# StandeHaas/Hydrodynamic-Limits-of-Active-Particle-Systems-with-Mean-Field-Interactions

Measured on AMD Instinct MI355X. Metric: particle-steps/sec at N=1e5, higher is better.
Workload: dtype f64; 1 GPU; BASELINE config 2: N=100000 particles, L=200000 sites, K=1, reflecting walls, sigma=0.005 (4001-tap table), beta=0.7, dt=0.0125, exclusion on; method=tiles

## Files before the change

hydrodynamic-limits-of-active-particle-systems-with-mean-field-interactions_amd/capi.py:

```python
from __future__ import annotations

import ctypes as C
import importlib.util
import os
import re
import sys

import numpy as np

HERE = os.path.dirname(os.path.abspath(__file__))
LIB_PATH = os.environ.get("APS_LIB") or os.path.join(HERE, "libaps_hip.so")
HEADER_PATH = os.path.join(os.path.dirname(HERE), "include", "aps.h")

APS_OK, APS_ERR_ARG, APS_ERR_HIP, APS_ERR_STATE, APS_ERR_NODEVICE = 0, -1, -2, -3, -4
METHODS = {"auto": 0, "pairs": 1, "lattice": 2, "tiles": 3}
KERNELS = ("pair_accumulate", "propose", "claim", "apply", "plan_tiles", "propose_lattice", "field_update", "tile_step")


class ApsError(RuntimeError):
    def __init__(self, code, text):
        super().__init__(f"libaps_hip error {code}: {text}")
        self.code = code


# ... 74 lines not shown
        "aps_observe_scalars": (C.c_int, [vp, i32, i32, i32, i32, vp, vp]),
        "aps_observe_scalars_all": (C.c_int, [vp, i32, vp, vp, vp]),
        "aps_event_overhead": (C.c_int, [vp, i32, P(dbl)]),
        "aps_observe_structure": (C.c_int, [vp, i32, i32, vp]),
        "aps_observe_bins": (C.c_int, [vp, i32, i32, vp, vp]),
        "aps_rates_from_field": (C.c_int, [vp, i32, vp, vp, vp, i64, vp, vp, vp, vp]),
        "aps_comm_unique_id": (C.c_int, [vp]),
        "aps_comm_init": (C.c_int, [vp, vp]),
        "aps_comm_ranks": (C.c_int, [vp, P(i32)]),
        "aps_owned_sites": (C.c_int, [vp, P(i32), P(i32)]),
        "aps_halo_copy": (C.c_int, [vp, vp]),
        "aps_halo_pack": (C.c_int, [vp, i32, vp, i64, P(i64)]),
        "aps_halo_unpack": (C.c_int, [vp, i32, vp, i64]),
        "aps_halo_info": (C.c_int, [vp, P(i32), P(i32), P(i32)]),
        "aps_comm_selftest": (C.c_int, [vp, i64]),
        "aps_halo_sizes": (C.c_int, [vp, P(i64), P(i64)]),
        "aps_ipc_export": (C.c_int, [vp, vp]),
        "aps_ipc_connect": (C.c_int, [vp, vp, vp]),
        "aps_exchange_kind": (C.c_int, [vp]),
        "aps_set_flip_table": (C.c_int, [vp, vp, i32]),
        "aps_ntt_info": (C.c_int, [vp, P(i32), P(i32), P(dbl), P(i64)]),
        "aps_ntt_launches": (C.c_int, [vp]),
        "aps_ntt_plan": (C.c_int, [i32, i32, i32, i32, P(i32), P(i32), P(i32)]),
        "aps_ntt_blocks": (C.c_int, [vp, P(i32), P(i32)]),
        "aps_tiles_info": (C.c_int, [vp, P(i32), P(i32), P(i32), P(i32)]),
    }
    lenient = os.environ.get("APS_LIB_LENIENT") == "1"
    for name, (res, args) in protos.items():
        if lenient and not hasattr(lib, name):
            continue
        fn = getattr(lib, name)
        fn.restype, fn.argtypes = res, args
    lib._aps_protos = protos
    _lib = lib
    return lib


def _ptr(a):
    return None if a is None else a.ctypes.data_as(C.c_void_p)


class Handle:

    def __init__(self, *, L, K, periodic, sigma_grid, rate_diffusion, rate_active, beta, dt, seed,
                 n_particles, minus_anchor=True, immobilize=True, suppress_flip=True, crowding=False,
                 k_on=0.0, k_off=0.0, k_exit=0.0, anchor_mask=None, device=0, rank=0, world=1,
# ... 274 lines not shown
        tlen, q = C.c_int32(), C.c_int32()
        self._ck(self.lib.aps_get_table(self._h, None, 0, C.byref(tlen), C.byref(q)))
        out = np.zeros(max(tlen.value, 1))
        self._ck(self.lib.aps_get_table(self._h, _ptr(out), len(out), C.byref(tlen), C.byref(q)))
        return out[:tlen.value], q.value

    def resort(self):
        self._ck(self.lib.aps_resort(self._h))


def device_count():
    return load().aps_device_count()


def ntt_plan(L, Rt, primes, max_log2=21):
    lib = load()
    nb, m, bs = C.c_int32(), C.c_int32(), C.c_int32()
    rc = lib.aps_ntt_plan(int(L), int(Rt), int(primes), int(max_log2), C.byref(nb), C.byref(m), C.byref(bs))
    if rc != APS_OK:
        raise ApsError(rc, lib.aps_last_error(None).decode())
    return dict(blocks=nb.value, log2_m=m.value, block_sites=bs.value)


def comm_unique_id() -> bytes:
    lib = load()
    buf = (C.c_uint8 * 128)()
    rc = lib.aps_comm_unique_id(C.cast(buf, C.c_void_p))
    if rc != APS_OK:
        raise ApsError(rc, lib.aps_last_error(None).decode())
    return bytes(buf)
```

hydrodynamic-limits-of-active-particle-systems-with-mean-field-interactions_amd/csrc/aps_common.hpp:

```cpp
#pragma once

#include <hip/hip_runtime.h>
#include <algorithm>
#include <cmath>
#include <cstdint>
#include <vector>

namespace {

__host__ __device__ inline double aps_exp(double x) {
    const double LOG2E = 0x1.71547652b82fep+0, LN2_HI = 0x1.62e42fee00000p-1, LN2_LO = 0x1.a39ef35793c76p-33;
    x = x > 700.0 ? 700.0 : (x < -700.0 ? -700.0 : x);
    const double kf = rint(x * LOG2E);
    double r = fma(-kf, LN2_HI, x);
    r = fma(-kf, LN2_LO, r);
    double p = 0x1.6124613a86d09p-33;
    p = fma(p, r, 0x1.1eed8eff8d898p-29);
    p = fma(p, r, 0x1.ae64567f544e4p-26);
    p = fma(p, r, 0x1.27e4fb7789f5cp-22);
    p = fma(p, r, 0x1.71de3a556c734p-19);
    p = fma(p, r, 0x1.a01a01a01a01ap-16);
    p = fma(p, r, 0x1.a01a01a01a01ap-13);
    p = fma(p, r, 0x1.6c16c16c16c17p-10);
    p = fma(p, r, 0x1.1111111111111p-7);
// ... 58 lines not shown
    const bool held = M.immobilize && !plus && anchored_site && bound;
    if (held) { act = 0.0; hl = 0.0; hr = 0.0; leave = M.k_exit; }
    double diff = hl + hr;
    if (!(plus && open_f)) act = 0.0;
    if (M.crowding) {
        double ff = 1.0 - (double)o_f / (double)K, fl = 1.0 - (double)o_l / (double)K, fr = 1.0 - (double)o_r / (double)K;
        ff = ff < 0.0 ? 0.0 : (ff > 1.0 ? 1.0 : ff);
        fl = fl < 0.0 ? 0.0 : (fl > 1.0 ? 1.0 : fl);
        fr = fr < 0.0 ? 0.0 : (fr > 1.0 ? 1.0 : fr);
        act *= ff;
        hl = M.rate_diffusion * (double)open_l * fl;
        hr = M.rate_diffusion * (double)open_r * fr;
        diff = hl + hr;
    }
    if (held) { diff = 0.0; act = 0.0; }
    Channels c;
    c.bind = (!bound && !plus && anchored_site && occ_self < K) ? M.k_on : 0.0;
    c.unbind = bound ? M.k_off : 0.0;
    c.diff = diff; c.act = act; c.flip = flip; c.leave = leave; c.left = hl; c.right = hr;
    c.total = ((((diff + act) + flip) + c.bind) + c.unbind) + leave;
    return c;
}

inline void weight_table(double sigma_grid, int L_, int K, bool periodic, std::vector<double> &table, int &tlen, int &q_out, int sum_bits = 51) {
    struct { double sigma_grid; int L, K; bool periodic; } p{sigma_grid, L_, K, periodic};
    table.clear();
    q_out = 0;
    if (!(p.sigma_grid > 0.0)) { tlen = 0; table.push_back(0.0); return; }
    const double s2 = p.sigma_grid * p.sigma_grid;
    const int64_t L = p.L;
    const int64_t lw = p.periodic ? L / 2 : (int64_t)(4.0 * p.sigma_grid + 0.5);
    const int64_t tmax = p.periodic ? L / 2 : std::min(lw, L);
    std::vector<double> w((size_t)tmax + 1);
    double wmax = 0.0;
    for (int64_t t = 0; t <= tmax; ++t) {
        double acc = 0.0;
        if (p.periodic) {
            const double a = (double)t;
            acc = aps_exp(-(0.5 * a * a) / s2);
        } else {
            for (int64_t k = 0;; ++k) {
                const int64_t d1 = t + 2 * L * k, d2 = 2 * L * k - t;
                bool any = false;
                if (d1 <= lw) { const double a = (double)d1; acc += aps_exp(-(0.5 * a * a) / s2); any = true; }
                if (k > 0 && d2 <= lw) { const double a = (double)d2; acc += aps_exp(-(0.5 * a * a) / s2); any = true; }
                if (!any) break;
// ... 65 lines not shown
```

hydrodynamic-limits-of-active-particle-systems-with-mean-field-interactions_amd/csrc/aps_hip.hip:

```cpp

#include <hip/hip_runtime.h>
#include <hip/hip_ext.h>
#include <dlfcn.h>
#include <unistd.h>
#include <rccl/rccl.h>
#include <algorithm>
#include <cmath>
#include <cstdint>
#include <cstdio>
#include <cstdlib>
#include <cstring>
#include <numeric>
#include <string>
#include <vector>

#include "aps.h"
#include "aps_common.hpp"
#include "dev_mem.hpp"

namespace {

constexpr uint32_t POS_MASK = 0x07FFFFFFu;
constexpr uint32_t SPIN_BIT = 1u << 27;
constexpr uint32_t BOUND_BIT = 1u << 28;
// ... 2020 lines not shown
template <bool F32>
const void *tl_kernel_f(bool periodic, int RS, bool k1) {
#define TL_PICK(BC, R) (k1 ? (const void *)&tile_loop<BC, R, true, F32> : (const void *)&tile_loop<BC, R, false, F32>)
#define TL_CASE(R) case R: return periodic ? TL_PICK(1, R) : TL_PICK(0, R);
    if (!F32 && (RS == 8 || (RS == 7 && !k1))) return nullptr;
#ifdef APS_DEV_RS
    switch (RS) { TL_CASE(APS_DEV_RS) default: return nullptr; }
#else
    if constexpr (F32) { if (RS == 8) return periodic ? TL_PICK(1, 8) : TL_PICK(0, 8); }
    switch (RS) {
        TL_CASE(1) TL_CASE(2) TL_CASE(3) TL_CASE(4) TL_CASE(5) TL_CASE(6)
        case 7: return k1 ? (periodic ? (const void *)&tile_loop<1, 7, true, F32> : (const void *)&tile_loop<0, 7, true, F32>)
                          : (F32 ? (periodic ? (const void *)&tile_loop<1, 7, false, true> : (const void *)&tile_loop<0, 7, false, true>) : nullptr);
        default: return nullptr;
    }
#endif
#undef TL_CASE
#undef TL_PICK
}
const void *tl_kernel(const aps_handle *h) {
    return h->f32 ? tl_kernel_f<true>(h->p.periodic != 0, h->ts_RS, h->p.K == 1) : tl_kernel_f<false>(h->p.periodic != 0, h->ts_RS, h->p.K == 1);
}

int loop_prepare(aps_handle *h) {
    if (h->loop_state != -2) return APS_OK;
    h->loop_state = 0;
    auto no = [&](const char *why) { h->loop_why = why; return APS_OK; };
    if (!is_tiles(h)) return no("not the tiles formulation");
    if (h->world != 1) return no("sharded handle");
    if (h->ntt_on) return no("field updated by the exact convolution");
    if (!h->ts_table_in_lds) return no("weight table beyond LDS");
    if (!h->model.field_mode) return no("global mean field");
    if (h->p.K == 1 && h->model.immobilize && h->model.k_exit > 0.0) return no("particles can leave the system (one cell per site)");
    if (3 * h->p.K > 32) return no("site capacity above 10");
    if (h->p.L - (int64_t)(h->ts_ntile - 1) * h->ts_own < 3) return no("last tile shorter than three sites");
#ifdef APS_STAMPS
    return no("diagnostic build");
#endif
    const void *fn = tl_kernel(h);
    if (!fn) return no("no kernel for this frame");
    const int64_t need_per_cu = ((int64_t)h->ts_ntile * h->E + h->num_cu - 1) / h->num_cu;
    h->loop_seg = 0;
    size_t lds_total = 0;
    for (int seg : {256, 192, 128, TL_SEG_MIN}) {
        const TlLds lay = tl_lds_layout(h->tlen, h->ts_RS, h->ts_own, h->p.K, ts_wbytes(h), seg);
        if (lay.total > 160 * 1024) continue;
// ... 469 lines not shown
        }
        if ((double)(((int64_t)p->L + 64 * 8 - 1) / (64 * 8)) * h->E > 8.0 * 256.0 && h->tlen <= 4096) h->fu_R = 7;
        if (const char *env = std::getenv("APS_FU_R")) { const int r = std::atoi(env); if (r >= 2 && r <= 8) h->fu_R = r; }
    }
    h->plan_interval = (!p->periodic && !(p->k_exit > 0.0)) ? 8 : 1;
    if (const char *env = std::getenv("APS_PLAN_INTERVAL")) h->plan_interval = std::max(1, std::atoi(env));

    auto die = [&](int code) { g_create_error = h->err; aps_destroy(h); return code; };
    if (hipSetDevice(p->device) != hipSuccess) { h->err = "hipSetDevice failed"; return die(APS_ERR_HIP); }
    if (hipStreamCreateWithFlags(&h->stream, hipStreamNonBlocking) != hipSuccess) { h->err = "hipStreamCreate failed"; return die(APS_ERR_HIP); }
    h->own_stream = true;
    int rc = set_lds_limit(h);
    if (rc) return die(rc);
    const size_t EN = (size_t)h->E * (size_t)h->Npad, EL = (size_t)h->E * (size_t)p->L;
    h->exit_cap = (int)std::max<int64_t>(h->N, 1);
    if ((rc = dev_alloc(h, &h->d_src, EN)) || (rc = dev_alloc(h, &h->d_orig, EN)) || (rc = dev_alloc(h, &h->d_prop_own, EN)) ||
        (rc = dev_alloc(h, &h->d_sp8, EN)) ||
        (rc = dev_alloc(h, &h->d_tinfo, (size_t)h->E * h->ntiles)) ||
        (rc = dev_alloc(h, &h->d_stamps, (size_t)8 * 4096)) ||
        (rc = dev_alloc(h, &h->d_plan, (size_t)h->E * h->ntiles * PLAN_CAP)) || (rc = dev_alloc(h, &h->d_plan_n, (size_t)h->E * h->ntiles)) ||
        (rc = dev_alloc(h, &h->d_accW, EN * MAX_SPLIT)) || (rc = dev_alloc(h, &h->d_accS, EN * MAX_SPLIT)) ||
        (rc = dev_alloc(h, &h->d_occ, EN * MAX_SPLIT)) || (rc = dev_alloc(h, &h->d_pcnt, 2 * EL)) ||
        (rc = dev_alloc(h, &h->d_plist, EL * 2 * p->K)) || (rc = dev_alloc(h, &h->d_table, h->table.size() + ((size_t)1 << h->bshift) + 8192))    ||
        (rc = dev_alloc(h, &h->d_beta, (size_t)h->E)) || (rc = dev_alloc(h, &h->d_gsum, (size_t)4 * h->E)) ||
        (rc = dev_alloc(h, &h->d_exit, (size_t)h->E * h->exit_cap * 3)) || (rc = dev_alloc(h, &h->d_nexit, (size_t)h->E)) ||
        (rc = dev_alloc(h, &h->d_mfield, (size_t)p->L)))
        return die(rc);
    h->d_prop = h->d_prop_own;
    if (h->method == APS_METHOD_LATTICE) {
        if ((rc = dev_alloc(h, &h->d_ws, EL)) || (rc = dev_alloc(h, &h->d_occ_site, EL)) ||
            (rc = dev_alloc(h, &h->d_dcnt, (size_t)h->E * h->nb)) || (rc = dev_alloc(h, &h->d_dep, (size_t)h->E * h->nb * h->dcap)) ||
            (rc = dev_alloc(h, &h->d_stepw, 2)))
            return die(rc);
    }
    if (h->method == APS_METHOD_TILES && h->world > 1 && (h->ts_kx < 1 || h->ts_kx * std::max(h->ts_reach, 1) > h->ts_ntile / h->world ||
                                                         (h->ts_ntile + h->world - 1) / h->world + 2 * (h->ts_kx - 1) * h->ts_reach > h->ts_ntile)) {
        h->err = "tiles, sharded: halo_interval " + std::to_string(h->ts_kx) + " x reach " + std::to_string(h->ts_reach) +
                 " tiles does not fit a rank's tile range (" + std::to_string(h->ts_ntile / h->world) + " tiles)";
        return die(APS_ERR_ARG);
    }
    if (h->method == APS_METHOD_TILES && h->world > 1 && 2 * h->ts_reach + 1 > h->ts_ntile / h->world) {
        h->err = "tiles, sharded: the table's reach (" + std::to_string(h->ts_reach) + " tiles) must stay below half a rank's tile range (" +
                 std::to_string(h->ts_ntile / h->world) + " tiles): fewer ranks or a larger lattice";
        return die(APS_ERR_ARG);
    }
    if (h->method == APS_METHOD_TILES) {
        const size_t ET = (size_t)h->E * h->ts_ntile;
// ... 19 lines not shown
            for (size_t i = 0; i < ti.size(); ++i) ti[i] = (int)std::ldexp(h->table[i], h->q);
            if ((rc = dev_alloc(h, &h->d_table_i, h->table.size() + ((size_t)1 << h->bshift) + 8192)) ||
                (rc = dev_alloc(h, &h->d_wsi[0], EL)) || (rc = dev_alloc(h, &h->d_wsi[1], EL))) return die(rc);
            if (hipMemcpyAsync(h->d_table_i, ti.data(), ti.size() * sizeof(int), hipMemcpyHostToDevice, h->stream) != hipSuccess ||
                hipStreamSynchronize(h->stream) != hipSuccess) { h->err = "integer table upload failed"; return die(APS_ERR_HIP); }
        }
        if ((rc = ntt_setup(h))) return die(rc);
        if (h->world > 1 && (rc = halo_setup(h))) return die(rc);
        const size_t need = ts_lds_layout(h->tlen, h->ts_table_in_lds, h->ts_RS, h->ts_own, p->K, ts_wbytes(h)).total;
        if (need > 160 * 1024) { h->err = "tiles: site capacity too large for the tile kernel's LDS staging"; return die(APS_ERR_ARG); }
        if (need > 48 * 1024 &&
            hipFuncSetAttribute(ts_kernel(p->periodic != 0, h->ts_table_in_lds, h->ts_RS, p->K == 1, h->f32), hipFuncAttributeMaxDynamicSharedMemorySize, (int)need) != hipSuccess) {
            h->err = "hipFuncSetAttribute(tile_step) failed"; return die(APS_ERR_HIP);
        }
    }
    if (p->anchor_mask) {
        if ((rc = dev_alloc(h, &h->d_anchor, (size_t)p->L))) return die(rc);
        if (hipMemcpyAsync(h->d_anchor, p->anchor_mask, (size_t)p->L, hipMemcpyHostToDevice, h->stream) != hipSuccess) { h->err = "anchor upload failed"; return die(APS_ERR_HIP); }
    }
    h->p.anchor_mask = nullptr;
    if (hipMemcpyAsync(h->d_table, h->table.data(), h->table.size() * sizeof(double), hipMemcpyHostToDevice, h->stream) != hipSuccess ||
        hipMemcpyAsync(h->d_beta, h->beta.data(), h->beta.size() * sizeof(double), hipMemcpyHostToDevice, h->stream) != hipSuccess ||
        hipStreamSynchronize(h->stream) != hipSuccess) { h->err = "table upload failed"; return die(APS_ERR_HIP); }
    *out = h;
    return APS_OK;
}

void aps_destroy(aps_handle *h) {
    if (!h) return;
    if (h->stream) (void)hipStreamSynchronize(h->stream);
    if (h->comm && g_rccl.CommDestroy) (void)g_rccl.CommDestroy(h->comm);
    for (hipEvent_t ev : h->events) (void)hipEventDestroy(ev);
    drop_graphs(h);
    if (h->cap_stream) (void)hipStreamDestroy(h->cap_stream);
    for (void *q : h->ipc_opened) if (q) (void)hipIpcCloseMemHandle(q);
    for (hipEvent_t ev : h->loop_ev) if (ev) (void)hipEventDestroy(ev);
    h->mem.free_all();
    if (h->own_stream && h->stream) (void)hipStreamDestroy(h->stream);
    delete h;
}

int aps_set_stream(aps_handle *h, void *hip_stream) {
    if (!h) return APS_ERR_ARG;
    HIP_TRY(h, hipStreamSynchronize(h->stream));
    if (h->own_stream && h->stream) { HIP_TRY(h, hipStreamDestroy(h->stream)); h->own_stream = false; }
    h->stream = reinterpret_cast<hipStream_t>(hip_stream);
// ... 385 lines not shown
    return APS_OK;
}

int aps_ntt_info(aps_handle *h, int32_t *on, int32_t *log2_m, double *prof_ms, int64_t *prof_launches) {
    if (!h) return APS_ERR_ARG;
    if (on) *on = h->ntt_on ? 1 : 0;
    if (log2_m) *log2_m = h->ntt_on ? h->ntt.m : 0;
    if (prof_ms) *prof_ms = h->prof_ntt_ms;
    if (prof_launches) *prof_launches = h->prof_ntt_n;
    return APS_OK;
}
int aps_ntt_plan(int32_t L, int32_t Rt, int32_t primes, int32_t max_log2, int32_t *blocks, int32_t *log2_m, int32_t *block_sites) {
    if (L < 2 || L > (1 << 25) || Rt < 0 || (primes != 1 && primes != 2)) {
        g_create_error = "aps_ntt_plan: 2 <= L <= 2^25, Rt >= 0, primes 1 or 2";
        return APS_ERR_ARG;
    }
    int nb, m, bs;
    ntt_plan_blocks(L, Rt, primes, max_log2, nb, m, bs);
    if (blocks) *blocks = nb;
    if (log2_m) *log2_m = m;
    if (block_sites) *block_sites = bs;
    return APS_OK;
}
int aps_ntt_blocks(aps_handle *h, int32_t *blocks, int32_t *block_sites) {
    if (!h) return APS_ERR_ARG;
    if (blocks) *blocks = h->ntt_on ? h->ntt.nb : 0;
    if (block_sites) *block_sites = h->ntt_on ? h->ntt.bs : 0;
    return APS_OK;
}
int aps_ntt_launches(aps_handle *h) {
    if (!h || !h->ntt_on) return 0;
    return h->ntt_fused ? 3 : h->ntt.a2 > 0 ? 5 : 3;
}

int aps_mark_reference(aps_handle *h, int32_t e) {
    if (!h) return APS_ERR_ARG;
    if (e < 0 || e >= h->E) return fail(h, APS_ERR_ARG, "aps_mark_reference: bad ensemble");
    if (h->n_set[(size_t)e] < 0) return fail(h, APS_ERR_STATE, "aps_mark_reference: no state uploaded for this ensemble");
    { int rc_ = sync_slots(h); if (rc_) return rc_; }
    int rc;
    if (!h->d_ref && (rc = dev_alloc(h, &h->d_ref, (size_t)h->E * h->Npad))) return rc;
    if (h->ref_set.empty()) h->ref_set.assign((size_t)h->E, 0);
    HIP_TRY(h, hipMemcpyAsync(h->d_ref + (size_t)e * h->Npad, h->d_src + (size_t)e * h->Npad, (size_t)h->Npad * 4, hipMemcpyDeviceToDevice, h->stream));
    HIP_TRY(h, hipStreamSynchronize(h->stream));
    h->ref_set[(size_t)e] = 1;
    return APS_OK;
// ... 311 lines not shown
            h->ipc_peer[side] = static_cast<char *>(ptr);
        }
        for (int par = 0; par < 2; ++par) h->ipc_peer_off[side][par] = (size_t)b[side].land_off[par][side];
    }
    h->ipc_on = true;
    return APS_OK;
}

int aps_set_flip_table(aps_handle *h, const double *table, int32_t n) {
    if (!h) return APS_ERR_ARG;
    HIP_TRY(h, hipStreamSynchronize(h->stream));
    if (h->graphs_built_f[0] || h->graphs_built_f[1]) drop_graphs(h);
    h->mem.release(h->d_flip_tab);
    h->d_flip_tab = nullptr;
    h->model.flip_tab = nullptr; h->model.flip_n = 0;
    if (table) {
        if (n < 1 || n > (1 << 24)) return fail(h, APS_ERR_ARG, "aps_set_flip_table: n must be in [1, 2^24]");
        for (int64_t i = 0; i < 2 * ((int64_t)n + 1); ++i)
            if (!(table[i] >= 0.0) || !std::isfinite(table[i])) return fail(h, APS_ERR_ARG, "aps_set_flip_table: rates must be finite and >= 0");
        HIP_TRY(h, h->mem.alloc(&h->d_flip_tab, (size_t)2 * ((size_t)n + 1)));
        HIP_TRY(h, hipMemcpy(h->d_flip_tab, table, (size_t)2 * ((size_t)n + 1) * sizeof(double), hipMemcpyHostToDevice));
        h->model.flip_tab = h->d_flip_tab; h->model.flip_n = n;
    }
    if (h->d_model) HIP_TRY(h, hipMemcpy(h->d_model, &h->model, sizeof(Model), hipMemcpyHostToDevice));
    return APS_OK;
}

int aps_tiles_info(aps_handle *h, int32_t *frame_sites, int32_t *owned_sites, int32_t *n_tiles, int32_t *table_in_lds) {
    if (!h) return APS_ERR_ARG;
    if (!is_tiles(h)) return fail(h, APS_ERR_STATE, "aps_tiles_info: not a tiles handle");
    if (frame_sites) *frame_sites = 64 * h->ts_RS;
    if (owned_sites) *owned_sites = h->ts_own;
    if (n_tiles) *n_tiles = h->ts_ntile;
    if (table_in_lds) *table_in_lds = h->ts_table_in_lds ? 1 : 0;
    return APS_OK;
}

int aps_exchange_kind(aps_handle *h) { return !h ? APS_ERR_ARG : (h->ipc_on ? 2 : (h->comm ? 1 : 0)); }

int aps_owned_sites(aps_handle *h, int32_t *lo, int32_t *hi) {
    if (!h) return APS_ERR_ARG;
    const bool sharded_sites = is_tiles(h) && h->world > 1;
    if (lo) *lo = sharded_sites ? h->own_lo : 0;
    if (hi) *hi = sharded_sites ? h->own_hi : h->p.L;
    return APS_OK;
}
// ... 250 lines not shown
```

hydrodynamic-limits-of-active-particle-systems-with-mean-field-interactions_amd/csrc/tile_loop.hpp:

```cpp
#pragma once

constexpr int TL_SEG_MIN = 88;
constexpr int TL_NG = 2;
#ifndef TL_MIN_WAVES
#define TL_MIN_WAVES 2
#endif
constexpr int TL_ABORT = 31;

struct LoopArgs {
    TileArgs a;
    unsigned long long step0;
    int nsteps;
    uint32_t tag0;
    int rec, drec;
    int seg;
    unsigned long long *xrec;
    unsigned *abort_dev, *abort_host;
    unsigned long long timeout_ticks;
#ifdef APS_LOOP_DEBUG
    uint32_t *dbg;
#endif
};

struct TlLds { size_t seg, cells, cells2, props, occ, misc, plist, fw, fs, tab, total; };
__host__ __device__ inline TlLds tl_lds_layout(int tlen, int RS, int own, int K, int wbytes, int seg) {
    TlLds l;
    const size_t TS = 64 * (size_t)RS, ncell = (TS + 2) * K;
    auto up = [](size_t v, size_t a) { return (v + a - 1) / a * a; };
    l.seg = 0;
    l.cells = l.seg + (size_t)FU_WAVES * 4 * (seg + 4) * sizeof(uint32_t);
    l.cells2 = up(l.cells + ncell * 4, 8);
    l.props = up(l.cells2 + (K == 1 ? 0 : ncell * 4), 8);
    l.occ = up(l.props + TS * K, 8);
    l.misc = up(l.occ + TS + 2, 8);
    l.plist = l.misc + 128;
    l.fw = up(l.plist + TS * (size_t)K * 8, 16);
    l.fs = l.fw + TS * wbytes;
    l.tab = up(l.fs + TS * wbytes, 16);
    l.total = l.tab + (size_t)ts_table_chunks(tlen, RS, own, wbytes) * 1024;
    return l;
}

typedef __attribute__((address_space(1))) unsigned long long tl_gu64;
typedef __attribute__((address_space(1))) unsigned tl_gu32;

__device__ __forceinline__ void tl_store_granule(unsigned long long *p, uint32_t tag, uint32_t word) {
    __hip_atomic_store((tl_gu64 *)p, ((unsigned long long)tag << 32) | word, __ATOMIC_RELAXED, __HIP_MEMORY_SCOPE_AGENT);
}
__device__ __forceinline__ unsigned long long tl_load_granule(const unsigned long long *p) {
    return __hip_atomic_load((tl_gu64 *)p, __ATOMIC_RELAXED, __HIP_MEMORY_SCOPE_AGENT);
}

__device__ __forceinline__ void tl_lds_add(double *p, double v) { unsafeAtomicAdd(p, v); }
__device__ __forceinline__ void tl_lds_add(int *p, int v) { atomicAdd(p, v); }

template <int BC, int RS, bool K1, bool F32>
__global__ __launch_bounds__(FU_THREADS, TL_MIN_WAVES) void tile_loop(const LoopArgs la, const void *__restrict__ table_v) {
    using W = typename TsField<F32>::w_t;
    using WS = typename TsField<F32>::ws_t;
    constexpr int SH = TsField<F32>::SH, WB = (int)sizeof(W);
    constexpr bool TAB_LDS = true;
    const TileArgs &a = la.a;
    const W *__restrict__ table_g = reinterpret_cast<const W *>(table_v);
    constexpr int TS = 64 * RS, NOLD = (TS + FU_THREADS - 1) / FU_THREADS;
    constexpr int NSLOT = 16, GB = FU_WAVES * 4;
    const int SEG = la.seg;
    extern __shared__ double lds[];
    const int L = a.L, K = K1 ? 1 : a.K, OWN = a.own;
    const TlLds lay = tl_lds_layout(a.tlen, RS, OWN, K, WB, la.seg);
    char *lds_c = reinterpret_cast<char *>(lds);
    uint32_t *seg_all = reinterpret_cast<uint32_t *>(lds_c + lay.seg);
    uint32_t *cellL = reinterpret_cast<uint32_t *>(lds_c + lay.cells);
    uint32_t *cellN = reinterpret_cast<uint32_t *>(lds_c + lay.cells2);
    uint8_t *propL = reinterpret_cast<uint8_t *>(lds_c + lay.props);
    uint8_t *occL = reinterpret_cast<uint8_t *>(lds_c + lay.occ);
    int *misc = reinterpret_cast<int *>(lds_c + lay.misc);
    uint2 *plist = reinterpret_cast<uint2 *>(lds_c + lay.plist);
    W *fieldW = reinterpret_cast<W *>(lds_c + lay.fw), *fieldS = reinterpret_cast<W *>(lds_c + lay.fs);
    W *tab = reinterpret_cast<W *>(lds_c + lay.tab);
    const int t = threadIdx.x, lane = t & 63, wave = __builtin_amdgcn_readfirstlane(t >> 6), e = blockIdx.y;
    const int tile = (int)blockIdx.x;
    const int own0 = tile * OWN, own_n = min(OWN, L - own0), nfr = own_n + 4;
    const int x0 = own0 - 2;
    const int x0c = max(x0, 0), x1c = min(x0 + nfr - 1, L - 1);
    const int Rt = a.tlen - 1;
    if (__hip_atomic_load((tl_gu32 *)la.abort_dev, __ATOMIC_RELAXED, __HIP_MEMORY_SCOPE_AGENT)) {
        if (t == 0) __hip_atomic_store(la.abort_host, 1u, __ATOMIC_RELAXED, __HIP_MEMORY_SCOPE_SYSTEM);
        return;
    }
    int n_iter = la.nsteps;
    {
        const unsigned stall = la.abort_dev[1];
        if (stall && (int)(stall >> 16) - 1 == tile && e == 0) n_iter = min(n_iter, (int)(stall & 0xFFFFu));
    }
    const uint32_t *__restrict__ cell_e = a.cell_in + (size_t)e * L * K;
    const WS *__restrict__ ws_e = reinterpret_cast<const WS *>(a.ws_in) + (size_t)e * L;
    const uint32_t *__restrict__ dcnt_e = a.dcnt_in + (size_t)e * a.ntile;
    const uint32_t *__restrict__ dep_e = a.dep_in + (size_t)e * a.ntile * a.dcap;
    uint32_t tbase = 0;
    {
        typedef __attribute__((address_space(3))) W lds_w;
        tbase = (uint32_t)(size_t)(lds_w *)tab;
    }
    if (t < 32) misc[t] = 0;
    {
        const int nchunk = ts_table_chunks(a.tlen, RS, OWN, WB);
        const char *srct = reinterpret_cast<const char *>(table_g) + lane * 16;
        for (int c = wave; c < nchunk; c += FU_WAVES) {
            const uint32_t m0v = (uint32_t)__builtin_amdgcn_readfirstlane((int)(tbase + (uint32_t)c * 1024u));
            asm volatile("s_mov_b32 m0, %0\n\tglobal_load_lds_dwordx4 %1, off" :: "s"(m0v), "v"(srct + c * 1024) : "memory");
        }
    }
    const double beta = a.beta[e];
    auto frame_site = [&](int i) -> int {
        if (i < -1 || i > nfr) return -1;
        int s = x0 + i;
        if (BC == 1) { s %= L; if (s < 0) s += L; return s; }
        return (s < 0 || s >= L) ? -1 : s;
    };
    const int ncell = (TS + 2) * K;
    for (int c = t; c < ncell; c += FU_THREADS) {
        const int s = frame_site(c / K - 1);
        const uint32_t v = cell_e[(unsigned)max(s, 0) * (unsigned)K + (unsigned)(c % K)];
        cellL[c] = s >= 0 ? v : CELL_EMPTY;
        if (!K1) cellN[c] = CELL_EMPTY;
    }
#pragma unroll
    for (int r = 0; r < NOLD; ++r) {
        const int xi = r * FU_THREADS + t;
        if (xi < TS) {
            const int s = xi < nfr ? frame_site(xi) : -1;
            WS o = ws_e[(unsigned)max(s, 0)];
            if (s < 0) { o.x = 0; o.y = 0; }
            fieldW[xi] = o.x; fieldS[xi] = o.y;
        }
    }
// ... 63 lines not shown
#define TLSTAMP(k)
#endif
    unsigned long long xg[TL_NG], xh = 0;
#pragma unroll
    for (int g = 0; g < TL_NG; ++g) xg[g] = 0;
    const int h_side = lane >> 5, h_i = lane & 31;
    const int h_nb = h_side ? nb_r : nb_l;
    const bool h_act = wave == FU_WAVES - 1 && h_i < 3 * K && h_nb >= 0;
    auto bucket_of = [&](int j, bool &ok) -> int {
        const int bi = j * GB + sub * FU_WAVES + wave;
        ok = j < ngroups && bi < nbk;
        int b = b0 + (ok ? bi : 0);
        if (b >= a.ntile) b -= a.ntile;
        return b;
    };
    for (int it = 0; it < n_iter; ++it) {
        const unsigned long long step = la.step0 + (unsigned long long)it;
        const uint32_t tag_in = la.tag0 + (uint32_t)it, tag_out = tag_in + 1u;
        const bool first = it == 0, last = it + 1 == la.nsteps;
        const unsigned long long *rec_in = la.xrec + ((size_t)((it + 1) & 1) * a.E * a.ntile + rec_e) * la.rec;
        unsigned long long *rec_out = la.xrec + ((size_t)(it & 1) * a.E * a.ntile + rec_e + tile) * la.rec;
        int *dcount = misc + (it & 1), *pcount = misc + 2 + (it & 1);
        bool gave_up = false;
        const int n0 = *pcount;
        uint2 mine = make_uint2(0u, CELL_EMPTY);
        uint32_t rx[4] = {0u, 0u, 0u, 0u};
        if (t < n0) {
            mine = plist[t];
            philox4x32_10((uint32_t)step, (uint32_t)(step >> 32), mine.y & CELL_ID, (uint32_t)(a.ens_base + e), a.seed_lo, a.seed_hi, rx);
        }
        TLSTAMP(2)
        auto spin_check = [&](unsigned &spins, unsigned long long &t_w) -> bool {
            __builtin_amdgcn_s_sleep(1);
            if ((++spins & 63u) != 0u) return false;
            const bool other = __hip_atomic_load((tl_gu32 *)la.abort_dev, __ATOMIC_RELAXED, __HIP_MEMORY_SCOPE_AGENT) != 0;
            const unsigned long long now = __builtin_amdgcn_s_memrealtime();
            if (!t_w) t_w = now;
            if (!other && now - t_w <= la.timeout_ticks) return false;
            if (!other && lane == 0) {
                __hip_atomic_store((tl_gu32 *)la.abort_dev, 1u, __ATOMIC_RELAXED, __HIP_MEMORY_SCOPE_AGENT);
                __hip_atomic_store(la.abort_host, 1u, __ATOMIC_RELAXED, __HIP_MEMORY_SCOPE_SYSTEM);
            }
            gave_up = true;
            return true;
        };
        auto wait_granule = [&](const unsigned long long *p, bool active) -> uint32_t {
            unsigned long long x = 0, t_w = 0;
            for (unsigned spins = 0;;) {
                if (active) x = tl_load_granule(p);
                if (!__ballot(active && (uint32_t)(x >> 32) != tag_in)) break;
                if (spin_check(spins, t_w)) break;
            }
// ... 6 lines not shown
#pragma unroll
                for (int g = 0; g < TL_NG; ++g) {
                    bool ok;
                    const int b = bucket_of(g, ok);
                    if (ok && (uint32_t)(xg[g] >> 32) != tag_in) {
                        xg[g] = tl_load_granule(rec_in + (size_t)b * la.rec + slot);
                        bad |= (uint32_t)(xg[g] >> 32) != tag_in;
                    }
                }
                if (h_act && (uint32_t)(xh >> 32) != tag_in) {
                    xh = tl_load_granule(rec_in + (size_t)h_nb * la.rec + la.drec + (h_side ? 0 : 3 * K) + h_i);
                    bad |= (uint32_t)(xh >> 32) != tag_in;
                }
                if (!__ballot(bad)) break;
                if (spin_check(spins, t_w)) break;
            }
            if (wave == FU_WAVES - 1 && !gave_up) {
                const uint32_t v = h_act ? (uint32_t)xh : CELL_EMPTY;
                const int hs = h_i / K, hk = h_i - hs * K, pos = (h_side ? own_n + 2 : -1) + hs;
                if (h_act) cellL[(h_side ? (own_n + 3) * K : 0) + h_i] = v;
                const unsigned long long mo = __ballot(h_act && v != CELL_EMPTY);
                if (h_i < 3 * K && hk == 0 && h_nb >= 0) occL[pos + 1] = (uint8_t)__popcll((mo >> (h_side * 32 + hs * K)) & ((1ull << K) - 1ull));
                const bool hp = h_act && v != CELL_EMPTY && pos >= 0 && pos < nfr;
                const unsigned long long mh = __ballot(hp);
                if (hp) plist[n0 + __builtin_amdgcn_mbcnt_hi((uint32_t)(mh >> 32), __builtin_amdgcn_mbcnt_lo((uint32_t)mh, 0u))] = make_uint2((uint32_t)pos | ((uint32_t)hk << 16), v);
                if (lane == 0) misc[4 + (it & 1)] = __popcll(mh);
            }
        }
        TLSTAMP(0)
        W accP[RS], accM[RS], accF[RS], accWi[RS], accSi[RS];
#pragma unroll
        for (int r = 0; r < RS; ++r) accP[r] = accM[r] = accF[r] = accWi[r] = accSi[r] = 0;
        uint32_t *shl = seg_all;
        const int CAP = (FU_WAVES * 4 * (SEG + 4) / 4) & ~3;
        unsigned long long *shcnt = reinterpret_cast<unsigned long long *>(misc + 8 + 2 * (it & 1));
        auto sweep_now = [&](unsigned long long m, const uint32_t word, const int cls) {
            while (m) {
                const int src_lane = __builtin_ctzll(m);
                m &= m - 1;
                const uint32_t e1 = (uint32_t)__builtin_amdgcn_readlane((int)word, src_lane);
                if (BC == 0) {
                    if (cls == 0) ts_one_abs<RS, 0, F32>(e1, x8, tb, accP);
                    else if (cls == 1) ts_one_abs<RS, 0, F32>(e1, x8, tb, accM);
                    else if (cls == 2) ts_one_abs<RS, 1, F32>(e1, x8, tb, accF);
                    else ts_image_group<TAB_LDS, RS, F32>(make_uint4(e1, DEP_NULL | ((uint32_t)x0c + TS_BIAS), DEP_NULL | ((uint32_t)x0c + TS_BIAS), DEP_NULL | ((uint32_t)x0c + TS_BIAS)),
                                                          x8, tb, table_g, tlen8, L8, accWi, accSi);
                } else {
                    const uint4 q = make_uint4(e1, DEP_NULL | ((uint32_t)null_site + TS_BIAS), DEP_NULL | ((uint32_t)null_site + TS_BIAS), DEP_NULL | ((uint32_t)null_site + TS_BIAS));
                    if (cls == 0) ts_group<1, TAB_LDS, RS, 0, F32>(q, x8, tb, table_g, tlen8, L8, accP);
// ... 121 lines not shown
            if (nI) {
                const uint32_t nulli = DEP_NULL | ((uint32_t)x0c + TS_BIAS);
                const uint4 *l4 = reinterpret_cast<const uint4 *>(shl + 3 * CAP);
#pragma unroll 1
                for (int g = rot & 3; g < (nI + 3) >> 2; g += FU_WAVES) {
                    uint4 q = l4[g];
                    if (4 * g + 1 >= nI) q.y = nulli;
                    if (4 * g + 2 >= nI) q.z = nulli;
                    if (4 * g + 3 >= nI) q.w = nulli;
                    ts_image_group<TAB_LDS, RS, F32>(q, x8, tb, table_g, tlen8, L8, accWi, accSi);
                }
            }
        }
        TLSTAMP(10)
#pragma unroll
        for (int r = 0; r < RS; ++r) {
            const W dw = (accP[r] + accM[r]) + accWi[r], ds = ((accP[r] - accM[r]) + accF[r]) + accSi[r];
            if (dw != 0) tl_lds_add(&fieldW[r * 64 + lane], dw);
            if (ds != 0) tl_lds_add(&fieldS[r * 64 + lane], ds);
        }
        TLSTAMP(11)
        __syncthreads();
        TLSTAMP(7)
        {
            const Model M = *a.model;
            const int n_part = n0 + misc[4 + (it & 1)];
            auto propose_one = [&](const uint2 pc, const uint32_t (&x)[4]) {
                const int pos = (int)(pc.x & 0xFFFFu), k = (int)(pc.x >> 16);
                const int s = frame_site(pos);
                const bool anch = a.anchor ? a.anchor[s] != 0 : false;
                propL[pos * K + k] = decide_proposal(M, anch, s, (pc.y & CELL_PLUS) ? 1 : -1, (pc.y & CELL_BOUND) != 0,
                                                     clip_field((double)fieldS[pos], (double)fieldW[pos]), beta, occL[pos + 1], occL[pos], occL[pos + 2], x);
            };
            if (t < n_part) {
                if (t >= n0) {
                    mine = plist[t];
                    philox4x32_10((uint32_t)step, (uint32_t)(step >> 32), mine.y & CELL_ID, (uint32_t)(a.ens_base + e), a.seed_lo, a.seed_hi, rx);
                }
                propose_one(mine, rx);
            }
            for (int j = FU_THREADS + t; j < n_part; j += FU_THREADS) {
                const uint2 pc = plist[j];
                uint32_t x[4];
                philox4x32_10((uint32_t)step, (uint32_t)(step >> 32), pc.y & CELL_ID, (uint32_t)(a.ens_base + e), a.seed_lo, a.seed_hi, x);
                propose_one(pc, x);
            }
        }
        __syncthreads();
        TLSTAMP(3)
        auto rank_at = [&](int j, uint32_t id) -> int {
            int n = 0;
            for (int k = 0; k < K; ++k) {
                const uint32_t cl_ = cellL[j * K + k], cr_ = cellL[(j + 2) * K + k];
                const int el = propL[(j - 1) * K + k] & 7, er = propL[(j + 1) * K + k] & 7;
                n += (cl_ != CELL_EMPTY && (el == EV_RIGHT || el == EV_FWD) && (cl_ & CELL_ID) < id);
                n += (cr_ != CELL_EMPTY && er == EV_LEFT && (cr_ & CELL_ID) < id);
            }
            return n;
        };
        auto cap_at = [&](int j) -> int { const int c = K - (int)occL[j + 1]; return c < 1 ? 1 : (c > 32 ? 32 : c); };
        auto put_deposit = [&](int kd, uint32_t d) { if (last) dep_o[kd] = d; else tl_store_granule(rec_out + kd, tag_out, d); };
        auto log_exit = [&](const uint32_t c, const int s) {
            const TileRare R = *a.rare;
            const unsigned kx = atomicAdd(&R.n_exit[e], 1u);
            if ((int)kx < R.exit_cap) {
                double *row = R.exit_log + ((size_t)e * R.exit_cap + kx) * 3;
                row[0] = (double)step; row[1] = (double)s; row[2] = (double)(c & CELL_ID);
            }
// ... 95 lines not shown
                    if (last) cell_o[(unsigned)frame_site(xi) * (unsigned)K + (unsigned)k] = c;
                    else {
                        if (io < 3) tl_store_granule(rec_out + la.drec + io * K + k, tag_out, c);
                        if (io >= own_n - 3) tl_store_granule(rec_out + la.drec + 3 * K + (io - (own_n - 3)) * K + k, tag_out, c);
                    }
                }
                if (!last) append(mine_site && c != CELL_EMPTY, xi, k, c, pnext);
            }
            if (mine_site) {
                occL[xi + 1] = (uint8_t)newn[r];
                if (last) {
                    WS f; f.x = fieldW[xi]; f.y = fieldS[xi];
                    reinterpret_cast<WS *>(a.ws_out)[(size_t)e * L + (unsigned)frame_site(xi)] = f;
                }
            }
        }
        if (!last && t < NSLOT) {
            const int idx = count + t;
            if (idx < (count / NSLOT + 1) * NSLOT && idx < la.drec) tl_store_granule(rec_out + idx, tag_out, DEP_NULL);
        }
        for (int i = t; i < (TS * K + 3) / 4; i += FU_THREADS) reinterpret_cast<uint32_t *>(propL)[i] = 0u;
        if (t == 0) {
            misc[(it + 1) & 1] = 0;
            misc[2 + (it & 1)] = 0; misc[4 + (it & 1)] = 0;
            misc[8 + 2 * (it & 1)] = 0; misc[9 + 2 * (it & 1)] = 0;
            if (last) {
                a.dcnt_out[(size_t)e * a.ntile + tile] = (uint32_t)count;
                if (tile == 0 && e == 0) a.stepw[(a.par + la.nsteps) & 1] = la.step0 + (unsigned long long)la.nsteps;
            }
        }
        if (!last) {
            const unsigned long long *rn = la.xrec + ((size_t)(it & 1) * a.E * a.ntile + rec_e) * la.rec;
#pragma unroll
            for (int g = 0; g < TL_NG; ++g) {
                bool ok;
                const int b = bucket_of(g, ok);
                xg[g] = ok ? tl_load_granule(rn + (size_t)b * la.rec + slot) : 0ull;
            }
            xh = h_act ? tl_load_granule(rn + (size_t)h_nb * la.rec + la.drec + (h_side ? 0 : 3 * K) + h_i) : 0ull;
        }
        TLSTAMP(5)
        __syncthreads();
    }
#ifdef APS_LOOP_STAMPS
    if (lane == 0 && tile < 512 && e == 0) {
        unsigned long long *o = a.rare->stamps + ((size_t)tile * FU_WAVES + wave) * 16;
        for (int k = 0; k < 12; ++k) o[k] = st_acc[k];
        o[6] = __builtin_amdgcn_s_memtime() - st_begin;
        o[1] = st_acc[8] + st_acc[9] + st_acc[10] + st_acc[11];
    }
#endif
}
```

include/aps.h:

```cpp
#ifndef APS_H
#define APS_H

#include <stdint.h>

#ifdef __cplusplus
extern "C" {
#endif

#define APS_OK 0
#define APS_ERR_ARG (-1)
#define APS_ERR_HIP (-2)
#define APS_ERR_STATE (-3)
#define APS_ERR_NODEVICE (-4)

typedef struct aps_handle aps_handle;

typedef struct aps_params {
    int32_t L;
    int32_t K;
    int32_t periodic;
    int32_t minus_anchor;
    int32_t immobilize;
    int32_t suppress_flip;
    int32_t crowding;
// ... 92 lines not shown

int aps_get_exits(aps_handle *h, int32_t ensemble, double *rows3, int64_t cap_rows, int64_t *n_rows);

int aps_get_table(aps_handle *h, double *out, int32_t cap, int32_t *tlen, int32_t *q);

int aps_resort(aps_handle *h);

int aps_step_timed(aps_handle *h, int64_t nsteps, double *kernel_ms, int64_t *launches, double *work);

int aps_step_info(aps_handle *h, int64_t *graph_steps, int64_t *single_steps);

int aps_set_flip_table(aps_handle *h, const double *table, int32_t n);

int aps_ntt_info(aps_handle *h, int32_t *on, int32_t *log2_m, double *prof_ms, int64_t *prof_launches);
int aps_ntt_plan(int32_t L, int32_t Rt, int32_t primes, int32_t max_log2, int32_t *blocks, int32_t *log2_m, int32_t *block_sites);
int aps_ntt_blocks(aps_handle *h, int32_t *blocks, int32_t *block_sites);
int aps_ntt_launches(aps_handle *h);

int aps_tiles_info(aps_handle *h, int32_t *frame_sites, int32_t *owned_sites, int32_t *n_tiles, int32_t *table_in_lds);

int aps_set_resident_loop(aps_handle *h, int32_t on);
int aps_loop_info(aps_handle *h, int64_t *loop_steps, int32_t *state, char *why, int32_t why_len);
int aps_step_loop_timed(aps_handle *h, int64_t nsteps, double *kernel_ms, int64_t *loop_steps);

int aps_copy_bandwidth(aps_handle *h, int64_t nbytes, int32_t reps, double *gbytes_per_s);

int aps_event_overhead(aps_handle *h, int32_t reps, double *ms_per_pair);

int aps_step_profile(aps_handle *h, int64_t nsteps, double *ms8, int64_t *launches8);

#ifdef __cplusplus
}
#endif
#endif
```

Before: 8.252 billion particle-steps/s.

## Prefilter particles by an upper-bound fire probability before proposing moves

```diff
diff --git a/hydrodynamic-limits-of-active-particle-systems-with-mean-field-interactions_amd/capi.py b/hydrodynamic-limits-of-active-particle-systems-with-mean-field-interactions_amd/capi.py
--- a/hydrodynamic-limits-of-active-particle-systems-with-mean-field-interactions_amd/capi.py
+++ b/hydrodynamic-limits-of-active-particle-systems-with-mean-field-interactions_amd/capi.py
@@ -120,6 +120,7 @@
         "aps_ntt_info": (C.c_int, [vp, P(i32), P(i32), P(dbl), P(i64)]),
         "aps_ntt_launches": (C.c_int, [vp]),
         "aps_ntt_plan": (C.c_int, [i32, i32, i32, i32, P(i32), P(i32), P(i32)]),
+        "aps_p_fire_bound": (C.c_int, [C.c_double] * 7 + [vp, i32, P(C.c_double)]),
         "aps_ntt_blocks": (C.c_int, [vp, P(i32), P(i32)]),
         "aps_tiles_info": (C.c_int, [vp, P(i32), P(i32), P(i32), P(i32)]),
     }
@@ -440,6 +441,17 @@
     return dict(blocks=nb.value, log2_m=m.value, block_sites=bs.value)
 
 
+def p_fire_bound(rate_diffusion, rate_active, k_on, k_off, k_exit, dt, beta, flip_table=None):
+    lib = load()
+    tab = None if flip_table is None else np.ascontiguousarray(flip_table, dtype=np.float64)
+    out = C.c_double()
+    rc = lib.aps_p_fire_bound(float(rate_diffusion), float(rate_active), float(k_on), float(k_off), float(k_exit), float(dt), float(beta),
+                              None if tab is None else _ptr(tab), 0 if tab is None else tab.shape[1] - 1, C.byref(out))
+    if rc != APS_OK:
+        raise ApsError(rc, lib.aps_last_error(None).decode())
+    return out.value
+
+
 def comm_unique_id() -> bytes:
     lib = load()
     buf = (C.c_uint8 * 128)()
diff --git a/hydrodynamic-limits-of-active-particle-systems-with-mean-field-interactions_amd/csrc/aps_common.hpp b/hydrodynamic-limits-of-active-particle-systems-with-mean-field-interactions_amd/csrc/aps_common.hpp
--- a/hydrodynamic-limits-of-active-particle-systems-with-mean-field-interactions_amd/csrc/aps_common.hpp
+++ b/hydrodynamic-limits-of-active-particle-systems-with-mean-field-interactions_amd/csrc/aps_common.hpp
@@ -104,6 +104,19 @@
     return c;
 }
 
+inline double p_fire_bound(const Model &M, double beta, const double *flip_host) {
+    auto pos = [](double v) { return v < 0.0 ? 0.0 : v; };
+    double f_max = std::exp(std::fabs(beta));
+    if (M.flip_n > 0 && flip_host) {
+        f_max = 0.0;
+        for (int64_t i = 0; i < 2 * ((int64_t)M.flip_n + 1); ++i) f_max = std::max(f_max, flip_host[i]);
+    }
+    const double t_max = 2.0 * pos(M.rate_diffusion) + pos(M.rate_active) + f_max + pos(M.k_on) + pos(M.k_off) + pos(M.k_exit);
+    const double margin = 1.0 + 0x1.0p-40;
+    const double p_hi = (1.0 - std::exp(-(t_max * pos(M.dt) * margin))) * margin + 0x1.0p-50;
+    return p_hi < 1.0 ? p_hi : 2.0;
+}
+
 inline void weight_table(double sigma_grid, int L_, int K, bool periodic, std::vector<double> &table, int &tlen, int &q_out, int sum_bits = 51) {
     struct { double sigma_grid; int L, K; bool periodic; } p{sigma_grid, L_, K, periodic};
     table.clear();
diff --git a/hydrodynamic-limits-of-active-particle-systems-with-mean-field-interactions_amd/csrc/aps_hip.hip b/hydrodynamic-limits-of-active-particle-systems-with-mean-field-interactions_amd/csrc/aps_hip.hip
--- a/hydrodynamic-limits-of-active-particle-systems-with-mean-field-interactions_amd/csrc/aps_hip.hip
+++ b/hydrodynamic-limits-of-active-particle-systems-with-mean-field-interactions_amd/csrc/aps_hip.hip
@@ -2066,6 +2066,13 @@
     return h->f32 ? tl_kernel_f<true>(h->p.periodic != 0, h->ts_RS, h->p.K == 1) : tl_kernel_f<false>(h->p.periodic != 0, h->ts_RS, h->p.K == 1);
 }
 
+int upload_p_hi(aps_handle *h, const double *flip_host) {
+    std::vector<double> p_hi((size_t)h->E);
+    for (int e = 0; e < h->E; ++e) p_hi[(size_t)e] = p_fire_bound(h->model, h->beta[(size_t)e], flip_host);
+    HIP_TRY(h, hipMemcpy(h->d_beta + h->E, p_hi.data(), p_hi.size() * sizeof(double), hipMemcpyHostToDevice));
+    return APS_OK;
+}
+
 int loop_prepare(aps_handle *h) {
     if (h->loop_state != -2) return APS_OK;
     h->loop_state = 0;
@@ -2581,7 +2588,7 @@
         (rc = dev_alloc(h, &h->d_accW, EN * MAX_SPLIT)) || (rc = dev_alloc(h, &h->d_accS, EN * MAX_SPLIT)) ||
         (rc = dev_alloc(h, &h->d_occ, EN * MAX_SPLIT)) || (rc = dev_alloc(h, &h->d_pcnt, 2 * EL)) ||
         (rc = dev_alloc(h, &h->d_plist, EL * 2 * p->K)) || (rc = dev_alloc(h, &h->d_table, h->table.size() + ((size_t)1 << h->bshift) + 8192))    ||
-        (rc = dev_alloc(h, &h->d_beta, (size_t)h->E)) || (rc = dev_alloc(h, &h->d_gsum, (size_t)4 * h->E)) ||
+        (rc = dev_alloc(h, &h->d_beta, (size_t)2 * h->E))    || (rc = dev_alloc(h, &h->d_gsum, (size_t)4 * h->E)) ||
         (rc = dev_alloc(h, &h->d_exit, (size_t)h->E * h->exit_cap * 3)) || (rc = dev_alloc(h, &h->d_nexit, (size_t)h->E)) ||
         (rc = dev_alloc(h, &h->d_mfield, (size_t)p->L)))
         return die(rc);
@@ -2647,6 +2654,7 @@
     if (hipMemcpyAsync(h->d_table, h->table.data(), h->table.size() * sizeof(double), hipMemcpyHostToDevice, h->stream) != hipSuccess ||
         hipMemcpyAsync(h->d_beta, h->beta.data(), h->beta.size() * sizeof(double), hipMemcpyHostToDevice, h->stream) != hipSuccess ||
         hipStreamSynchronize(h->stream) != hipSuccess) { h->err = "table upload failed"; return die(APS_ERR_HIP); }
+    if ((rc = upload_p_hi(h, nullptr))) return die(rc);
     *out = h;
     return APS_OK;
 }
@@ -3078,6 +3086,15 @@
     if (block_sites) *block_sites = bs;
     return APS_OK;
 }
+int aps_p_fire_bound(double rate_diffusion, double rate_active, double k_on, double k_off, double k_exit, double dt, double beta,
+                     const double *flip_table, int32_t flip_n, double *p_hi) {
+    if (!p_hi || flip_n < 0 || (flip_n > 0 && !flip_table)) { g_create_error = "aps_p_fire_bound: null argument"; return APS_ERR_ARG; }
+    Model M{};
+    M.rate_diffusion = rate_diffusion; M.rate_active = rate_active; M.k_on = k_on; M.k_off = k_off; M.k_exit = k_exit; M.dt = dt;
+    M.flip_n = flip_n;
+    *p_hi = p_fire_bound(M, beta, flip_table);
+    return APS_OK;
+}
 int aps_ntt_blocks(aps_handle *h, int32_t *blocks, int32_t *block_sites) {
     if (!h) return APS_ERR_ARG;
     if (blocks) *blocks = h->ntt_on ? h->ntt.nb : 0;
@@ -3435,6 +3452,7 @@
         HIP_TRY(h, hipMemcpy(h->d_flip_tab, table, (size_t)2 * ((size_t)n + 1) * sizeof(double), hipMemcpyHostToDevice));
         h->model.flip_tab = h->d_flip_tab; h->model.flip_n = n;
     }
+    if (int rc = upload_p_hi(h, table)) return rc;
     if (h->d_model) HIP_TRY(h, hipMemcpy(h->d_model, &h->model, sizeof(Model), hipMemcpyHostToDevice));
     return APS_OK;
 }
diff --git a/hydrodynamic-limits-of-active-particle-systems-with-mean-field-interactions_amd/csrc/tile_loop.hpp b/hydrodynamic-limits-of-active-particle-systems-with-mean-field-interactions_amd/csrc/tile_loop.hpp
--- a/hydrodynamic-limits-of-active-particle-systems-with-mean-field-interactions_amd/csrc/tile_loop.hpp
+++ b/hydrodynamic-limits-of-active-particle-systems-with-mean-field-interactions_amd/csrc/tile_loop.hpp
@@ -4,6 +4,9 @@
 constexpr int TL_NG = 2;
 #ifndef TL_MIN_WAVES
 #define TL_MIN_WAVES 2
+#endif
+#ifndef TL_ROT_SHIFT
+#define TL_ROT_SHIFT 8
 #endif
 constexpr int TL_ABORT = 31;
 
@@ -22,7 +25,7 @@
 #endif
 };
 
-struct TlLds { size_t seg, cells, cells2, props, occ, misc, plist, fw, fs, tab, total; };
+struct TlLds { size_t seg, cells, cells2, props, occ, misc, plist, sv_x, sv_pc, fw, fs, tab, total; };
 __host__ __device__ inline TlLds tl_lds_layout(int tlen, int RS, int own, int K, int wbytes, int seg) {
     TlLds l;
     const size_t TS = 64 * (size_t)RS, ncell = (TS + 2) * K;
@@ -34,7 +37,9 @@
     l.occ = up(l.props + TS * K, 8);
     l.misc = up(l.occ + TS + 2, 8);
     l.plist = l.misc + 128;
-    l.fw = up(l.plist + TS * (size_t)K * 8, 16);
+    l.sv_x = up(l.plist + TS * (size_t)K * 8, 16);
+    l.sv_pc = l.sv_x + TS * (size_t)K * 16;
+    l.fw = up(l.sv_pc + TS * (size_t)K * 8, 16);
     l.fs = l.fw + TS * wbytes;
     l.tab = up(l.fs + TS * wbytes, 16);
     l.total = l.tab + (size_t)ts_table_chunks(tlen, RS, own, wbytes) * 1024;
@@ -76,6 +81,8 @@
     uint8_t *occL = reinterpret_cast<uint8_t *>(lds_c + lay.occ);
     int *misc = reinterpret_cast<int *>(lds_c + lay.misc);
     uint2 *plist = reinterpret_cast<uint2 *>(lds_c + lay.plist);
+    uint4 *sv_x = reinterpret_cast<uint4 *>(lds_c + lay.sv_x);
+    uint2 *sv_pc = reinterpret_cast<uint2 *>(lds_c + lay.sv_pc);
     W *fieldW = reinterpret_cast<W *>(lds_c + lay.fw), *fieldS = reinterpret_cast<W *>(lds_c + lay.fs);
     W *tab = reinterpret_cast<W *>(lds_c + lay.tab);
     const int t = threadIdx.x, lane = t & 63, wave = __builtin_amdgcn_readfirstlane(t >> 6), e = blockIdx.y;
@@ -112,6 +119,8 @@
         }
     }
     const double beta = a.beta[e];
+    const double p_hi = a.beta[a.E + e];
+    const int prop_wave = (tile + (tile >> TL_ROT_SHIFT)) & (FU_WAVES - 1);
     auto frame_site = [&](int i) -> int {
         if (i < -1 || i > nfr) return -1;
         int s = x0 + i;
@@ -221,12 +230,30 @@
         unsigned long long *rec_out = la.xrec + ((size_t)(it & 1) * a.E * a.ntile + rec_e + tile) * la.rec;
         int *dcount = misc + (it & 1), *pcount = misc + 2 + (it & 1);
         bool gave_up = false;
-        const int n0 = *pcount;
-        uint2 mine = make_uint2(0u, CELL_EMPTY);
-        uint32_t rx[4] = {0u, 0u, 0u, 0u};
-        if (t < n0) {
-            mine = plist[t];
-            philox4x32_10((uint32_t)step, (uint32_t)(step >> 32), mine.y & CELL_ID, (uint32_t)(a.ens_base + e), a.seed_lo, a.seed_hi, rx);
+        const int n0 = __builtin_amdgcn_readfirstlane(*pcount);
+        auto draw = [&](const uint2 pc, uint32_t (&x)[4]) -> bool {
+            philox4x32_10((uint32_t)step, (uint32_t)(step >> 32), pc.y & CELL_ID, (uint32_t)(a.ens_base + e), a.seed_lo, a.seed_hi, x);
+            const double u0 = ((double)(x[0] >> 5) * 67108864.0 + (double)(x[1] >> 6)) * 0x1.0p-53;
+            return u0 < p_hi;
+        };
+        auto survive = [&](bool sv, const uint2 pc, const uint32_t (&x)[4]) {
+            const unsigned long long mm = __ballot(sv);
+            const int cnt_u = __popcll(mm);
+            int base = 0;
+            if (lane == 0 && cnt_u) base = atomicAdd(misc + 6, cnt_u);
+            base = __builtin_amdgcn_readfirstlane(base);
+            if (sv) {
+                const int i = base + (int)__builtin_amdgcn_mbcnt_hi((uint32_t)(mm >> 32), __builtin_amdgcn_mbcnt_lo((uint32_t)mm, 0u));
+                sv_pc[i] = pc; sv_x[i] = make_uint4(x[0], x[1], x[2], x[3]);
+            }
+        };
+        for (int j0 = wave * 64; j0 < n0; j0 += FU_THREADS) {
+            const int j = j0 + lane;
+            uint2 pc = make_uint2(0u, CELL_EMPTY);
+            uint32_t x[4] = {0u, 0u, 0u, 0u};
+            bool sv = false;
+            if (j < n0) { pc = plist[j]; sv = draw(pc, x); }
+            survive(sv, pc, x);
         }
         TLSTAMP(2)
         auto spin_check = [&](unsigned &spins, unsigned long long &t_w) -> bool {
@@ -279,9 +306,11 @@
                 const unsigned long long mo = __ballot(h_act && v != CELL_EMPTY);
                 if (h_i < 3 * K && hk == 0 && h_nb >= 0) occL[pos + 1] = (uint8_t)__popcll((mo >> (h_side * 32 + hs * K)) & ((1ull << K) - 1ull));
                 const bool hp = h_act && v != CELL_EMPTY && pos >= 0 && pos < nfr;
-                const unsigned long long mh = __ballot(hp);
-                if (hp) plist[n0 + __builtin_amdgcn_mbcnt_hi((uint32_t)(mh >> 32), __builtin_amdgcn_mbcnt_lo((uint32_t)mh, 0u))] = make_uint2((uint32_t)pos | ((uint32_t)hk << 16), v);
-                if (lane == 0) misc[4 + (it & 1)] = __popcll(mh);
+                const uint2 hpc = make_uint2((uint32_t)pos | ((uint32_t)hk << 16), v);
+                uint32_t hx[4] = {0u, 0u, 0u, 0u};
+                bool hsv = false;
+                if (hp) hsv = draw(hpc, hx);
+                survive(hsv, hpc, hx);
             }
         }
         TLSTAMP(0)
@@ -449,9 +478,10 @@
         TLSTAMP(11)
         __syncthreads();
         TLSTAMP(7)
-        {
+        const int nsv = __builtin_amdgcn_readfirstlane(misc[6]);
+        const int sv0 = ((wave - prop_wave) & (FU_WAVES - 1)) * 64;
+        if (sv0 < nsv) {
             const Model M = *a.model;
-            const int n_part = n0 + misc[4 + (it & 1)];
             auto propose_one = [&](const uint2 pc, const uint32_t (&x)[4]) {
                 const int pos = (int)(pc.x & 0xFFFFu), k = (int)(pc.x >> 16);
                 const int s = frame_site(pos);
@@ -459,18 +489,10 @@
                 propL[pos * K + k] = decide_proposal(M, anch, s, (pc.y & CELL_PLUS) ? 1 : -1, (pc.y & CELL_BOUND) != 0,
                                                      clip_field((double)fieldS[pos], (double)fieldW[pos]), beta, occL[pos + 1], occL[pos], occL[pos + 2], x);
             };
-            if (t < n_part) {
-                if (t >= n0) {
-                    mine = plist[t];
-                    philox4x32_10((uint32_t)step, (uint32_t)(step >> 32), mine.y & CELL_ID, (uint32_t)(a.ens_base + e), a.seed_lo, a.seed_hi, rx);
-                }
-                propose_one(mine, rx);
-            }
-            for (int j = FU_THREADS + t; j < n_part; j += FU_THREADS) {
-                const uint2 pc = plist[j];
-                uint32_t x[4];
-                philox4x32_10((uint32_t)step, (uint32_t)(step >> 32), pc.y & CELL_ID, (uint32_t)(a.ens_base + e), a.seed_lo, a.seed_hi, x);
-                propose_one(pc, x);
+            for (int j = sv0 + lane; j < nsv; j += FU_THREADS) {
+                const uint4 x4 = sv_x[j];
+                const uint32_t x[4] = {x4.x, x4.y, x4.z, x4.w};
+                propose_one(sv_pc[j], x);
             }
         }
         __syncthreads();
@@ -612,7 +634,7 @@
         for (int i = t; i < (TS * K + 3) / 4; i += FU_THREADS) reinterpret_cast<uint32_t *>(propL)[i] = 0u;
         if (t == 0) {
             misc[(it + 1) & 1] = 0;
-            misc[2 + (it & 1)] = 0; misc[4 + (it & 1)] = 0;
+            misc[2 + (it & 1)] = 0; misc[6] = 0;
             misc[8 + 2 * (it & 1)] = 0; misc[9 + 2 * (it & 1)] = 0;
             if (last) {
                 a.dcnt_out[(size_t)e * a.ntile + tile] = (uint32_t)count;
@@ -638,6 +660,8 @@
         for (int k = 0; k < 12; ++k) o[k] = st_acc[k];
         o[6] = __builtin_amdgcn_s_memtime() - st_begin;
         o[1] = st_acc[8] + st_acc[9] + st_acc[10] + st_acc[11];
+        o[12] = 1ull + (unsigned)__builtin_amdgcn_s_getreg(4 | (31 << 11));
+        o[13] = (unsigned)__builtin_amdgcn_s_getreg(20 | (31 << 11));
     }
 #endif
 }
diff --git a/include/aps.h b/include/aps.h
--- a/include/aps.h
+++ b/include/aps.h
@@ -138,6 +138,8 @@
 int aps_set_resident_loop(aps_handle *h, int32_t on);
 int aps_loop_info(aps_handle *h, int64_t *loop_steps, int32_t *state, char *why, int32_t why_len);
 int aps_step_loop_timed(aps_handle *h, int64_t nsteps, double *kernel_ms, int64_t *loop_steps);
+int aps_p_fire_bound(double rate_diffusion, double rate_active, double k_on, double k_off, double k_exit, double dt, double beta,
+                     const double *flip_table, int32_t flip_n, double *p_hi);
 
 int aps_copy_bandwidth(aps_handle *h, int64_t nbytes, int32_t reps, double *gbytes_per_s);
 
```

New measurement: 7.982 billion particle-steps/s. -3.3%, worse.
